# csiro-icvg/Diff3DHPE

Hardware: AMD Instinct MI355X
Metric: pose_sequences_per_sec (higher is better)
Workload: dtype f16x3

## Files before the change

diff3dhpe_amd/csrc/kernels_qkv_sattn.hip:

```cpp
#include "d3d_kernels.h"
#include "qkv_fused_kloop.h"

#include <math.h>

namespace d3d {
namespace {

#include "kloop_common.h"
#include "attn_lds.h"

QF_SHAPE(8, 3, 256, 192, 4, 3);
constexpr int QS_J = 17, QS_FPT = 15, QS_ROWS = QS_J * QS_FPT;
constexpr int QS_PLANE = QS_J * 128, QS_SLOT = 6 * QS_PLANE;
constexpr int QS_QKV = QF_STAGE;
constexpr int QS_STX = QS_QKV + 8 * QS_SLOT;
constexpr int QS_RAW = 2 * QF_STAGE;
constexpr int QS_RAW_MAX = 16384;
constexpr int QS_LDS = QS_STX + QF_BM * 8;
static_assert(QS_LDS <= 160 * 1024 && QS_RAW + QS_RAW_MAX <= QS_STX, "LDS map");
constexpr int QS_PV = 0, QS_PK = 2 * QS_PLANE, QS_PQ = 4 * QS_PLANE;

#ifndef QS_ABL
#define QS_ABL 0
#endif

struct QsArgs {
  const _Float16* Ap;
  const _Float16* Wp;
  const float* bias;
  const float* csum;
  const float* st_in;
  int st_np;
  float eps, out_scale;
  _Float16* out;
  int M, K, F, mtiles, D;
  unsigned* range;
  _Float16 *ph, *pl;
};

__device__ __forceinline__ void qs_attention(unsigned char* slot, int lane, _Float16* out_row0, int D) {
  constexpr int T = QS_J;
  unsigned char* const sVh = slot + QS_PV;
  unsigned char* const sVl = slot + QS_PV + QS_PLANE;
  unsigned char* const sKh = slot + QS_PK;
  unsigned char* const sKl = slot + QS_PK + QS_PLANE;
  unsigned char* const sQh = slot + QS_PQ;
  unsigned char* const sQl = slot + QS_PQ + QS_PLANE;
  unsigned char* const patch = slot + QS_PQ;
  const int r = lane & 31, h = lane >> 5;
  h8 qh[4], ql[4];
#pragma unroll
  for (int ks = 0; ks < 4; ++ks) {
    const int qo = kswz(r, 2 * ks + h);
    qh[ks] = *reinterpret_cast<const h8*>(sQh + qo);
    ql[ks] = *reinterpret_cast<const h8*>(sQl + qo);
  }
  f32x16 sacc;
#pragma unroll
  for (int q = 0; q < 16; ++q) sacc[q] = 0.f;
#pragma unroll
  for (int ks = 0; ks < 4; ++ks) {
    const int ko = kswz(r, 2 * ks + h);
    const h8 kh = *reinterpret_cast<const h8*>(sKh + ko);
    const h8 kl = *reinterpret_cast<const h8*>(sKl + ko);
    sacc = __builtin_amdgcn_mfma_f32_32x32x16_f16(kl, qh[ks], sacc, 0, 0, 0);
    sacc = __builtin_amdgcn_mfma_f32_32x32x16_f16(kh, ql[ks], sacc, 0, 0, 0);
    sacc = __builtin_amdgcn_mfma_f32_32x32x16_f16(kh, qh[ks], sacc, 0, 0, 0);
  }
  float m = -INFINITY;
  if (h != 0) sacc[8] = -INFINITY;
#pragma unroll
  for (int q = 0; q < 9; ++q) m = fmaxf(m, sacc[q]);
  m = fmaxf(m, __shfl_xor(m, 32, 64));
  constexpr float C_EXP = 1.4426950408889634f / 64.0f;
  const float mb = m * C_EXP;
  float l = 0.f;
#pragma unroll
  for (int q = 0; q < 16; ++q) {
    float e = 0.0f;
    if (q < 9) {
      e = __builtin_amdgcn_exp2f(fmaf(sacc[q], C_EXP, -mb));
      l += e;
    }
    sacc[q] = e;
  }
  l += __shfl_xor(l, 32, 64);
  f32x16 oacc[2];
#pragma unroll
  for (int q = 0; q < 16; ++q) { oacc[0][q] = 0.f; oacc[1][q] = 0.f; }
#pragma unroll
  for (int s2 = 0; s2 < 2; ++s2) {
    h8 eh, el;
    {
      if (s2 == 0) {
        float e8[8];
#pragma unroll
        for (int jj = 0; jj < 8; ++jj) e8[jj] = sacc[jj];
        split8_e(e8, eh, el);
      } else {
        unsigned a, b;
        split_pair_s(sacc[8], 0.0f, 1024.0f, a, b);
        u32x4 hv = {a, 0u, 0u, 0u}, lv = {b, 0u, 0u, 0u};
        eh = __builtin_bit_cast(h8, hv);
        el = __builtin_bit_cast(h8, lv);
      }
    }
    const int k0 = 16 * s2 + 4 * h;
    const int gi = lane & 15, tq_ = gi >> 2, tp_ = gi & 3;
#pragma unroll
    for (int dt = 0; dt < 2; ++dt) {
      const int d0 = dt * 32 + 16 * ((lane >> 4) & 1);
      const int ch = (d0 >> 3) + (tp_ >> 1), sub = (tp_ & 1) * 8;
      const int o0 = vswz(k0 + tq_, ch) + sub, o1 = vswz(k0 + 8 + tq_, ch) + sub;
      const s4v a0 = __builtin_amdgcn_ds_read_tr16_b64_v4i16((__attribute__((address_space(3))) s4v*)(uintptr_t)(sVh + o0));
      const s4v a1 = __builtin_amdgcn_ds_read_tr16_b64_v4i16((__attribute__((address_space(3))) s4v*)(uintptr_t)(sVh + o1));
      const s4v c0 = __builtin_amdgcn_ds_read_tr16_b64_v4i16((__attribute__((address_space(3))) s4v*)(uintptr_t)(sVl + o0));
      const s4v c1 = __builtin_amdgcn_ds_read_tr16_b64_v4i16((__attribute__((address_space(3))) s4v*)(uintptr_t)(sVl + o1));
      h8 vh, vl;
      {
        const h4 a0h = __builtin_bit_cast(h4, a0), a1h = __builtin_bit_cast(h4, a1);
        const h4 c0h = __builtin_bit_cast(h4, c0), c1h = __builtin_bit_cast(h4, c1);
#pragma unroll
        for (int e = 0; e < 4; ++e) { vh[e] = a0h[e]; vh[4 + e] = a1h[e]; vl[e] = c0h[e]; vl[4 + e] = c1h[e]; }
      }
      oacc[dt] = __builtin_amdgcn_mfma_f32_32x32x16_f16(vl, eh, oacc[dt], 0, 0, 0);
      oacc[dt] = __builtin_amdgcn_mfma_f32_32x32x16_f16(vh, el, oacc[dt], 0, 0, 0);
      oacc[dt] = __builtin_amdgcn_mfma_f32_32x32x16_f16(vh, eh, oacc[dt], 0, 0, 0);
    }
    __builtin_amdgcn_sched_barrier(0);
  }
  const float inv = 1.0f / (8192.0f * l);
  const int tqc = r < T ? r : 0;
  u32x4 pw[6];
#pragma unroll
  for (int dt = 0; dt < 2; ++dt) {
#pragma unroll
    for (int g4 = 0; g4 < 4; ++g4) {
      const int vo = vswz(tqc, dt * 4 + g4) + 8 * h;
      const uint2 vqh = *reinterpret_cast<const uint2*>(sVh + vo);
      const uint2 vql = *reinterpret_cast<const uint2*>(sVl + vo);
      float o4[4];
#pragma unroll
      for (int pr = 0; pr < 2; ++pr) {
        const unsigned ph_ = pr ? vqh.y : vqh.x, pl_ = pr ? vql.y : vql.x;
        float n0, n1;
        asm("v_fma_mix_f32 %0, %1, %2, 0 op_sel_hi:[1,0,0]" : "=v"(n0) : "v"(pl_), "v"(-0.125f));
        asm("v_fma_mix_f32 %0, %1, %2, %3 op_sel_hi:[1,0,0]" : "=v"(n0) : "v"(ph_), "v"(-0.125f), "v"(n0));
        asm("v_fma_mix_f32 %0, %1, %2, 0 op_sel:[1,0,0] op_sel_hi:[1,0,0]" : "=v"(n1) : "v"(pl_), "v"(-0.125f));
        asm("v_fma_mix_f32 %0, %1, %2, %3 op_sel:[1,0,0] op_sel_hi:[1,0,0]" : "=v"(n1) : "v"(ph_), "v"(-0.125f), "v"(n1));
        o4[2 * pr] = __builtin_fmaf(oacc[dt][4 * g4 + 2 * pr], inv, n0);
        o4[2 * pr + 1] = __builtin_fmaf(oacc[dt][4 * g4 + 2 * pr + 1], inv, n1);
      }
      unsigned h0, l0, h1, l1;
      split_pair(o4[0], o4[1], 8.0f, h0, l0);
      split_pair(o4[2], o4[3], 8.0f, h1, l1);
      const h4 oh = __builtin_bit_cast(h4, make_uint2(h0, h1)), ol = __builtin_bit_cast(h4, make_uint2(l0, l1));
      if (!(QS_ABL & 4)) patch_wr(patch, r, h, g4, oh, ol);
      else asm volatile("" ::"v"(oh), "v"(ol));
    }
    asm volatile("" ::: "memory");
#pragma unroll
    for (int it = 0; it < 3; ++it) pw[dt * 3 + it] = (QS_ABL & 4) ? u32x4{0u, 0u, 0u, 0u} : patch_rd(patch, 8 * it + (lane >> 3), lane & 7);
    asm volatile("" ::: "memory");
  }
  _Float16* const pw_ptr = out_row0 + (size_t)(lane >> 3) * 2 * D + 8 * (lane & 7);
  const size_t pw_stride = (size_t)8 * 2 * D;
#pragma unroll
  for (int it = 0; it < 3; ++it)
    if (8 * it + (lane >> 3) < T) {
#pragma unroll
      for (int dt = 0; dt < 2; ++dt) *reinterpret_cast<u32x4*>(pw_ptr + it * pw_stride + dt * 64) = pw[dt * 3 + it];
    }
}

typedef float qs_f2 __attribute__((ext_vector_type(2)));

__device__ __forceinline__ void qs_row_stats(unsigned char* lds, const QsArgs& a, int m0, int wave, int lane, bool st_dma) {
  float2* const srow = reinterpret_cast<float2*>(lds + QS_STX);
  const int K = a.K;
  if (lane < 32) {
    const int t = wave * 32 + lane, row = m0 + t;
    float sm = 0.f, sq = 0.f;
    if (row < a.M) {
      const float2* raw = st_dma ? reinterpret_cast<const float2*>(lds + QS_RAW) + t * a.st_np
                                 : reinterpret_cast<const float2*>(a.st_in) + (size_t)row * a.st_np;
      for (int p = 0; p < a.st_np; ++p) { sm += raw[p].x; sq += raw[p].y; }
    }
    if (sq >= (X3_HALF_MAX * 0.125f) * (X3_HALF_MAX * 0.125f)) range_raise(a.range, RANGE_BIT_ACT);
    const float mean = sm / (float)K;
    const float var = fmaxf(sq / (float)K - mean * mean, 0.0f);
    if (row < a.M && mean * mean > 256.0f * var) range_raise(a.range, RANGE_BIT_STATS);
    const float rstd = 1.0f / sqrtf(var + a.eps);
    srow[t] = make_float2(rstd * a.out_scale, -mean * rstd);
  }
}

__device__ __forceinline__ void qs_fold_split(const f32x4& ac, qs_f2 sx, qs_f2 sy, const float4& cs, const float4& bb, float osc, float& amax,
                                              u32x2_alias& hv, u32x2_alias& lv) {
  typedef qs_f2 f2;
  f2 a01, a23, c01, c23, b01, b23;
  a01.x = ac[0]; a01.y = ac[1]; a23.x = ac[2]; a23.y = ac[3];
  c01.x = cs.x; c01.y = cs.y; c23.x = cs.z; c23.y = cs.w;
  b01.x = bb.x; b01.y = bb.y; b23.x = bb.z; b23.y = bb.w;
  const f2 v01 = __builtin_elementwise_fma(sx, a01, __builtin_elementwise_fma(sy, c01, b01));
  const f2 v23 = __builtin_elementwise_fma(sx, a23, __builtin_elementwise_fma(sy, c23, b23));
  amax = fmaxf(fmaxf(amax, fabsf(v01.x)), fabsf(v01.y));
  amax = fmaxf(fmaxf(amax, fabsf(v23.x)), fabsf(v23.y));
  unsigned h0, l0, h1, l1;
  split_pair(v01.x, v01.y, osc, h0, l0);
  split_pair(v23.x, v23.y, osc, h1, l1);
  hv[0] = h0; hv[1] = h1; lv[0] = l0; lv[1] = l1;
}

template <bool PLANES>
__device__ __forceinline__ void qs_tail(f32x4 (&acc)[QF_TM][QF_NJ], unsigned char* lds, const QsArgs& a, int mt, int hd, int m0, int n0,
                                        int wave, int lane, int wm, int wn, int r16, int q) {
  float2 st[QF_TM];
#pragma unroll
  for (int i = 0; i < QF_TM; ++i) st[i] = reinterpret_cast<const float2*>(lds + QS_STX)[wm * 16 * QF_TM + 16 * i + r16];
  float4 cs4[QF_NJ], b4[QF_NJ];
#pragma unroll
  for (int j = 0; j < QF_NJ; ++j) {
    const int n = n0 + wn * 48 + 16 * j + 4 * q;
    cs4[j] = *reinterpret_cast<const float4*>(a.csum + n);
    b4[j] = *reinterpret_cast<const float4*>(a.bias + n);
  }
  float amaxj[QF_NJ] = {0.0f, 0.0f, 0.0f};
  typedef qs_f2 f2;
  const int chunk = 2 * wn + (q >> 1), half8 = (q & 1) << 3;
  auto write_pass = [&](int pass) {
#pragma unroll
    for (int i = 0; i < QF_TM; ++i) {
      if (pass == 0 ? (i > 4) : (i < 4 && !(wm == 1 && i == 0))) continue;
      const int R = wm * 16 * QF_TM + 16 * i + r16;
      const int fr = (R * 241) >> 12, jr = R - fr * QS_J;
      if (((fr >> 2) & 1) != pass || fr >= QS_FPT) continue;
      unsigned char* const row = lds + QS_QKV + ((fr & 3) + 4 * (fr >> 3)) * QS_SLOT + jr * 128 + half8;
      unsigned char* const pkq = row + ((chunk ^ ((jr >> 1) & 7)) << 4);
      unsigned char* const pv = row + ((chunk ^ vkey(jr)) << 4);
      const f2 sx = (f2)(st[i].x), sy = (f2)(st[i].y);
#pragma unroll
      for (int j = 0; j < QF_NJ; ++j) {
        const float osc = j == 0 ? 1.0f : 8.0f;
        u32x2_alias hv, lv;
        qs_fold_split(acc[i][j], sx, sy, cs4[j], b4[j], osc, amaxj[j], hv, lv);
        unsigned char* const ph = j == 0 ? pkq + QS_PQ : (j == 1 ? pkq + QS_PK : pv + QS_PV);
        if (!(QS_ABL & 1)) {
          *reinterpret_cast<u32x2_alias*>(ph) = hv;
          *reinterpret_cast<u32x2_alias*>(ph + QS_PLANE) = lv;
        }
      }
    }
  };
  auto attend = [&](int pass) {
    const int fr = (wave & 3) + 4 * pass + 8 * (wave >> 2);
    const long long gf = (long long)mt * QS_FPT + fr;
    if (!(QS_ABL & 2) && fr < QS_FPT && gf < a.F)
      qs_attention(lds + QS_QKV + wave * QS_SLOT, lane, a.out + ((size_t)gf * QS_J) * 2 * a.D + hd * 128, a.D);
  };
  auto range_check = [&]() {
    float amax = 0.0f;
#pragma unroll
    for (int j = 0; j < QF_NJ; ++j) amax = fmaxf(amax, amaxj[j] * (j == 0 ? 1.0f : (j == 1 ? 8.0f : 16.015f)));
    if (amax > X3_HALF_MAX) range_raise(a.range, RANGE_BIT_ACT);
  };
  if (PLANES) {
#pragma unroll
    for (int i = 0; i < QF_TM; ++i) {
      const int R = wm * 16 * QF_TM + 16 * i + r16, m = m0 + R;
      if (R >= QS_ROWS || m >= a.M) continue;
      const f2 sx = (f2)(st[i].x), sy = (f2)(st[i].y);
      const size_t o = (size_t)m * 3 * a.D + hd * 64 + 16 * wn + 4 * q;
#pragma unroll
      for (int j = 0; j < QF_NJ; ++j) {
        const float osc = j == 0 ? 1.0f : 8.0f;
        u32x2_alias hv, lv;
        qs_fold_split(acc[i][j], sx, sy, cs4[j], b4[j], osc, amaxj[j], hv, lv);
        *reinterpret_cast<u32x2_alias*>(a.ph + o + j * a.D) = hv;
        *reinterpret_cast<u32x2_alias*>(a.pl + o + j * a.D) = lv;
      }
    }
    range_check();
    return;
  }
  write_pass(0);
  __syncthreads();
  attend(0);
  __syncthreads();
  write_pass(1);
  range_check();
  __syncthreads();
  attend(1);
}

__global__ __launch_bounds__(512) void k_qkv_sattn(QsArgs a) {
  extern __shared__ __attribute__((aligned(16))) unsigned char lds[];
  const int G = (int)gridDim.x, b = (int)blockIdx.x;
  const int tiles = a.mtiles * 8;
  if (b >= tiles) return;
  const int nitems = (tiles - b + G - 1) / G;
  const int vfull = (a.mtiles / 8) * 64, mrem = a.mtiles % 8;
  auto tile_of = [&](int o, int& mt, int& hd) {
    if (o < vfull) {
      const int xcd = o & 7, slot = o >> 3;
      mt = (slot >> 3) * 8 + xcd;
      hd = slot & 7;
    } else {
      const int o2 = o - vfull;
      mt = (a.mtiles / 8) * 8 + o2 % mrem;
      hd = o2 / mrem;
    }
  };

  const int K = a.K;
  const size_t K2 = 2 * (size_t)K;
  const int nk = K / 32;
  int mt = 0, hd = 0;
  tile_of(b, mt, hd);
  QF_STAGE_FIRST(a.Ap, a.Wp, mt * QS_ROWS, hd * QF_BN)
  int tid_o = (int)threadIdx.x;
  for (int item = 0; item < nitems; ++item) {
    QF_TILE_LANES;
    QF_TILE_NEXT(mtn, hdn);
    const int m0 = mt * QS_ROWS, n0 = hd * QF_BN;

    const int st_bytes = QF_BM * a.st_np * 8;
    const bool st_dma = st_bytes <= QS_RAW_MAX && (((size_t)m0 * a.st_np * 8) & 15) == 0;
    int st_issued = 0;
    if (st_dma) {
      const char* src = reinterpret_cast<const char*>(a.st_in + (size_t)m0 * a.st_np * 2);
#pragma unroll
      for (int it = 0; it < QS_RAW_MAX / 1024 / 8; ++it) {
        const int pc = wave + it * 8;
        if (pc * 1024 < st_bytes) {
          KL_GLDS(sgpr_ptr(src + pc * 1024) + lane * 16, QS_RAW + pc * 1024);
          ++st_issued;
        }
      }
    }

    QF_TILE_PLAN(a.Ap, a.Wp, m0, n0, mtn * QS_ROWS, hdn * QF_BN);
    QF_TILE_ACC;
    int issued_prev = st_issued;
    QF_KLOOP_HEAD(QF_PIECE)
    qs_row_stats(lds, a, m0, wave, lane, st_dma);
    QF_KLOOP_TAIL(QF_PIECE)
    __builtin_amdgcn_s_setprio(0);

    __syncthreads();

    qs_tail<false>(acc, lds, a, mt, hd, m0, n0, wave, lane, wm, wn, r16, q);
    mt = mtn; hd = hdn;
    __syncthreads();
  }
}

struct QdSrc {
  const float *x2d, *y;
  const float *G, *P, *Q;
  int q_stride;
  int TJ, y_bcast_T;
};
constexpr int QD_GROW = 8;
constexpr int QD_QSLOTS = 16;
constexpr int QD_G = 0, QD_P = QD_G + QF_BN * QD_GROW * 4, QD_Q = QD_P + QS_J * QF_BN * 4;
static_assert(QD_Q + QD_QSLOTS * QF_BN * 4 <= QS_QKV, "the direct form's tables fit the unused stage area");
static_assert(QF_BM <= QD_QSLOTS * QS_J, "a tile's rows span at most QD_QSLOTS frames, so at most QD_QSLOTS batch elements");

__device__ __forceinline__ int qd_col(int c, int hd) { return 512 * ((c % 48) >> 4) + 64 * hd + 16 * (c / 48) + (c & 15); }

template <int CIN2>
__device__ __forceinline__ void qd_stage(unsigned char* lds, const QdSrc& d, int M, int m0, int hd, int tid) {
  constexpr int CIN = CIN2 + 3;
  float* const sG = reinterpret_cast<float*>(lds + QD_G);
  float* const sP = reinterpret_cast<float*>(lds + QD_P);
  float* const sQ = reinterpret_cast<float*>(lds + QD_Q);
  for (int idx = tid; idx < QF_BN * CIN; idx += 512) {
    const int c = idx / CIN, k = idx - c * CIN;
    sG[c * QD_GROW + k] = d.G[QF_BN * CIN * hd + idx];
  }
  for (int idx = tid; idx < QS_J * QF_BN; idx += 512) {
    const int j = idx / QF_BN, c = idx - j * QF_BN;
    sP[idx] = d.P[j * 1536 + QF_BN * hd + c];
  }
  if (d.Q) {
    const int b_lo = m0 / d.TJ, nb = d.q_stride ? min(QD_QSLOTS, M / d.TJ - b_lo) : 1;
    for (int idx = tid; idx < nb * QF_BN; idx += 512) {
      const int sl = idx / QF_BN, c = idx - sl * QF_BN;
      sQ[idx] = d.Q[(size_t)(b_lo + sl) * d.q_stride + qd_col(c, hd)];
    }
  }
}

template <int CIN2>
__device__ __forceinline__ void qd_fill(f32x4 (&acc)[QF_TM][QF_NJ], const unsigned char* lds, const QdSrc& d, int M, int m0, int wm, int wn,
                                        int r16, int q) {
  constexpr int CIN = CIN2 + 3;
  const int c0 = wn * 48 + 4 * q;
  const int b_lo = m0 / d.TJ;
  const float* const sG = reinterpret_cast<const float*>(lds + QD_G);
  const float* const sP = reinterpret_cast<const float*>(lds + QD_P);
  const float* const sQ = reinterpret_cast<const float*>(lds + QD_Q);
  float u[QF_TM][CIN];
#pragma unroll
  for (int ii = 0; ii < QF_TM; ++ii) {
    const int R = wm * 16 * QF_TM + 16 * ii + r16, m = m0 + R;
    const int fr = (R * 241) >> 12, jr = R - fr * QS_J;
#pragma unroll
    for (int k = 0; k < CIN; ++k) u[ii][k] = 0.0f;
    if (m < M) {
#pragma unroll
      for (int k = 0; k < CIN2; ++k) u[ii][k] = d.x2d[(size_t)m * CIN2 + k];
      const size_t my = d.y_bcast_T ? ((size_t)(m / d.TJ) * QS_J + jr) : (size_t)m;
#pragma unroll
      for (int k = 0; k < 3; ++k) u[ii][CIN2 + k] = d.y[my * 3 + k];
    }
  }
#pragma unroll
  for (int j = 0; j < QF_NJ; ++j) {
#pragma unroll
    for (int e = 0; e < 4; ++e) {
      float g[CIN];
#pragma unroll
      for (int k = 0; k < CIN; ++k) g[k] = sG[(c0 + 16 * j + e) * QD_GROW + k];
#pragma unroll
      for (int ii = 0; ii < QF_TM; ++ii) {
        float v = 0.0f;
#pragma unroll
        for (int k = 0; k < CIN; ++k) v = fmaf(u[ii][k], g[k], v);
        acc[ii][j][e] = v;
      }
      __builtin_amdgcn_sched_barrier(0);
    }
  }
#pragma unroll
  for (int i = 0; i < QF_TM; ++i) {
    const int R = wm * 16 * QF_TM + 16 * i + r16, m = m0 + R;
    const int po = (R - ((R * 241) >> 12) * QS_J) * QF_BN + c0;
    const int qo = c0 + (d.q_stride ? min(m / d.TJ - b_lo, QD_QSLOTS - 1) * QF_BN : 0);
    if (m < M) {
#pragma unroll
      for (int j = 0; j < QF_NJ; ++j) {
        const float4 p4 = *reinterpret_cast<const float4*>(sP + po + 16 * j);
        acc[i][j][0] += p4.x; acc[i][j][1] += p4.y; acc[i][j][2] += p4.z; acc[i][j][3] += p4.w;
      }
      if (d.Q) {
#pragma unroll
        for (int j = 0; j < QF_NJ; ++j) {
          const float4 q4 = *reinterpret_cast<const float4*>(sQ + qo + 16 * j);
          acc[i][j][0] += q4.x; acc[i][j][1] += q4.y; acc[i][j][2] += q4.z; acc[i][j][3] += q4.w;
        }
      }
    }
    __builtin_amdgcn_sched_barrier(0);
  }
}

template <int CIN2, bool PLANES>
__global__ __launch_bounds__(512) void k_qkv_sattn_direct(QsArgs a, QdSrc d) {
  extern __shared__ __attribute__((aligned(16))) unsigned char lds[];
  const int G = (int)gridDim.x, b = (int)blockIdx.x;
  const int tiles = a.mtiles * 8;
  if (b >= tiles) return;
  const int nitems = (tiles - b + G - 1) / G;
  KL_XCD_TILE_ORDER(a.mtiles, 8);
  int tid_o = (int)threadIdx.x;
  for (int item = 0; item < nitems; ++item) {
    QF_TILE_LANES;
    int mt = 0, hd = 0;
    tile_of(item * G + b, mt, hd);
    const int m0 = mt * QS_ROWS, n0 = hd * QF_BN;
    qd_stage<CIN2>(lds, d, a.M, m0, hd, tid);
    qs_row_stats(lds, a, m0, wave, lane, false);
    __syncthreads();
    f32x4 acc[QF_TM][QF_NJ];
    qd_fill<CIN2>(acc, lds, d, a.M, m0, wm, wn, r16, q);
    __builtin_amdgcn_sched_barrier(0);
    qs_tail<PLANES>(acc, lds, a, mt, hd, m0, n0, wave, lane, wm, wn, r16, q);
    __syncthreads();
  }
}

}

bool qkv_sattn_ok(int J, int D, int H, int K) { return J == QS_J && H == 8 && D == 512 && K % 64 == 0 && K >= 128; }

hipError_t launch_qkv_sattn(const void* Apair, const void* Wpair_headmajor, const float* bias_hm, const float* csum_hm, const float* st_in,
                            int st_np, float eps, int w_exp, void* out_x3, int M, int K, int J, int D, int H, hipStream_t s) {
  if (!qkv_sattn_ok(J, D, H, K) || M <= 0 || M % J != 0 || st_np < 1 || !Apair || !Wpair_headmajor || !bias_hm || !csum_hm || !st_in || !out_x3)
    return hipErrorInvalidValue;
  if (w_exp < -14 || w_exp > 12) return hipErrorInvalidValue;
  QsArgs a{};
  a.Ap = (const _Float16*)Apair; a.Wp = (const _Float16*)Wpair_headmajor; a.bias = bias_hm; a.csum = csum_hm; a.st_in = st_in;
  a.st_np = st_np; a.eps = eps; a.out_scale = ldexpf(1.0f, -(3 + w_exp));
  a.out = (_Float16*)out_x3; a.M = M; a.K = K; a.F = M / J; a.mtiles = (a.F + QS_FPT - 1) / QS_FPT; a.D = D;
  a.range = launch_range_word();
  int grid = 0;
  if (hipError_t ge = persistent_grid((long long)a.mtiles * 8, grid)) return ge;
  return launch_lds<k_qkv_sattn>(dim3(grid), dim3(512), QS_LDS, s, a);
}

bool qkv_sattn_direct_ok(int J, int D, int H, int in_chans) { return qkv_sattn_ok(J, D, H, D) && in_chans >= 1 && in_chans <= 3; }

hipError_t launch_qkv_sattn_direct(const float* x2d, const float* y, int y_bcast_T, int in_chans, const float* G, const float* P, const float* Q,
                                   int q_stride, const float* bias_hm, const float* csum_hm, const float* st_in, int st_np, float eps, void* out_x3,
                                   void* planes_hi, void* planes_lo, int M, int T, int J, int D, int H, hipStream_t s) {
  if (!qkv_sattn_direct_ok(J, D, H, in_chans) || M <= 0 || T <= 0 || M % (T * J) != 0 || st_np < 1 || !x2d || !y || !G || !P || !bias_hm || !csum_hm ||
      !st_in || (q_stride != 0 && q_stride != 3 * D) || (!out_x3 && (!planes_hi || !planes_lo)))
    return hipErrorInvalidValue;
  QsArgs a{};
  a.bias = bias_hm; a.csum = csum_hm; a.st_in = st_in; a.st_np = st_np; a.eps = eps; a.out_scale = 1.0f;
  a.out = (_Float16*)out_x3; a.M = M; a.K = D; a.F = M / J; a.mtiles = (a.F + QS_FPT - 1) / QS_FPT; a.D = D;
  a.ph = (_Float16*)planes_hi; a.pl = (_Float16*)planes_lo;
  a.range = launch_range_word();
  QdSrc d{};
  d.x2d = x2d; d.y = y; d.G = G; d.P = P; d.Q = Q; d.q_stride = q_stride; d.TJ = T * J; d.y_bcast_T = y_bcast_T;
  int grid = 0;
  if (hipError_t ge = persistent_grid((long long)a.mtiles * 8, grid)) return ge;
#define D3D_QD(C2)                                                                                                      \
  case C2:                                                                                                              \
    return out_x3 ? launch_lds<k_qkv_sattn_direct<C2, false>>(dim3(grid), dim3(512), QS_LDS, s, a, d)                   \
                  : launch_lds<k_qkv_sattn_direct<C2, true>>(dim3(grid), dim3(512), QS_LDS, s, a, d);
  switch (in_chans) {
    D3D_QD(1) D3D_QD(2) D3D_QD(3)
  }
#undef D3D_QD
  return hipErrorInvalidValue;
}

}
```

Baseline: 136.1.

## Prefetch direct-form inputs into double-buffered LDS via async global-to-LDS loads

The direct QKV kernel now issues global_load_lds requests for the next tile's x2d, y and row-statistic partials into one of two LDS input buffers while the current tile computes. qd_fill and qs_row_stats then read those inputs from LDS instead of global memory. Per-head G/P tables are restaged only when the head changes, and the broadcast Q row is split from the per-batch Q rows. The goal is to hide global load latency and cut redundant table reloads, at the cost of more LDS use, clamped index logic and a wait_vm(0) that drains every outstanding load each iteration.

```diff
diff --git a/diff3dhpe_amd/csrc/kernels_qkv_sattn.hip b/diff3dhpe_amd/csrc/kernels_qkv_sattn.hip
--- a/diff3dhpe_amd/csrc/kernels_qkv_sattn.hip
+++ b/diff3dhpe_amd/csrc/kernels_qkv_sattn.hip
@@ -175,14 +175,14 @@
 
 typedef float qs_f2 __attribute__((ext_vector_type(2)));
 
-__device__ __forceinline__ void qs_row_stats(unsigned char* lds, const QsArgs& a, int m0, int wave, int lane, bool st_dma) {
+__device__ __forceinline__ void qs_row_stats(unsigned char* lds, const QsArgs& a, int m0, int wave, int lane, bool st_dma, int raw_off = QS_RAW) {
   float2* const srow = reinterpret_cast<float2*>(lds + QS_STX);
   const int K = a.K;
   if (lane < 32) {
     const int t = wave * 32 + lane, row = m0 + t;
     float sm = 0.f, sq = 0.f;
     if (row < a.M) {
-      const float2* raw = st_dma ? reinterpret_cast<const float2*>(lds + QS_RAW) + t * a.st_np
+      const float2* raw = st_dma ? reinterpret_cast<const float2*>(lds + raw_off) + t * a.st_np
                                  : reinterpret_cast<const float2*>(a.st_in) + (size_t)row * a.st_np;
       for (int p = 0; p < a.st_np; ++p) { sm += raw[p].x; sq += raw[p].y; }
     }
@@ -364,13 +364,22 @@
 constexpr int QD_GROW = 8;
 constexpr int QD_QSLOTS = 16;
 constexpr int QD_G = 0, QD_P = QD_G + QF_BN * QD_GROW * 4, QD_Q = QD_P + QS_J * QF_BN * 4;
-static_assert(QD_Q + QD_QSLOTS * QF_BN * 4 <= QS_QKV, "the direct form's tables fit the unused stage area");
+constexpr int QD_STNP_MAX = 2;
+constexpr int QD_IN = QD_Q + QD_QSLOTS * QF_BN * 4;
+constexpr int QD_IN_X = 0, QD_IN_Y = QD_IN_X + QF_BM * 3 * 4, QD_IN_ST = QD_IN_Y + QF_BM * 3 * 4;
+constexpr int QD_IN_BYTES = QD_IN_ST + QF_BM * QD_STNP_MAX * 8;
+static_assert(QD_IN + 2 * QD_IN_BYTES <= QS_QKV, "the direct form's tables and input buffers fit the unused stage area");
+static_assert(QS_QKV + 8 * QS_SLOT <= QS_STX && QS_STX + QF_BM * 8 <= QS_LDS, "frame slots and row statistics lie behind them");
+static_assert(QD_IN % 16 == 0 && QD_IN_BYTES % 16 == 0 && QD_IN_Y % 16 == 0 && QD_IN_ST % 16 == 0, "input blocks start on 16 bytes");
 static_assert(QF_BM <= QD_QSLOTS * QS_J, "a tile's rows span at most QD_QSLOTS frames, so at most QD_QSLOTS batch elements");
 
+#define QD_GLDS4(SRC, DSTOFF)                                                                                            \
+  __builtin_amdgcn_global_load_lds(reinterpret_cast<const char*>(SRC), (__attribute__((address_space(3))) void*)(uintptr_t)(lds + (DSTOFF)), 4, 0, 0)
+
 __device__ __forceinline__ int qd_col(int c, int hd) { return 512 * ((c % 48) >> 4) + 64 * hd + 16 * (c / 48) + (c & 15); }
 
 template <int CIN2>
-__device__ __forceinline__ void qd_stage(unsigned char* lds, const QdSrc& d, int M, int m0, int hd, int tid) {
+__device__ __forceinline__ void qd_stage_tables(unsigned char* lds, const QdSrc& d, int hd, int tid) {
   constexpr int CIN = CIN2 + 3;
   float* const sG = reinterpret_cast<float*>(lds + QD_G);
   float* const sP = reinterpret_cast<float*>(lds + QD_P);
@@ -383,37 +392,70 @@
     const int j = idx / QF_BN, c = idx - j * QF_BN;
     sP[idx] = d.P[j * 1536 + QF_BN * hd + c];
   }
-  if (d.Q) {
-    const int b_lo = m0 / d.TJ, nb = d.q_stride ? min(QD_QSLOTS, M / d.TJ - b_lo) : 1;
-    for (int idx = tid; idx < nb * QF_BN; idx += 512) {
-      const int sl = idx / QF_BN, c = idx - sl * QF_BN;
-      sQ[idx] = d.Q[(size_t)(b_lo + sl) * d.q_stride + qd_col(c, hd)];
-    }
+  if (d.Q && !d.q_stride && tid < QF_BN) sQ[tid] = d.Q[qd_col(tid, hd)];
+}
+
+__device__ __forceinline__ void qd_stage_q_rows(unsigned char* lds, const QdSrc& d, int M, int m0, int hd, int tid) {
+  float* const sQ = reinterpret_cast<float*>(lds + QD_Q);
+  const int b_lo = m0 / d.TJ, nb = min(QD_QSLOTS, M / d.TJ - b_lo);
+  for (int idx = tid; idx < nb * QF_BN; idx += 512) {
+    const int sl = idx / QF_BN, c = idx - sl * QF_BN;
+    sQ[idx] = d.Q[(size_t)(b_lo + sl) * d.q_stride + qd_col(c, hd)];
   }
 }
 
 template <int CIN2>
-__device__ __forceinline__ void qd_fill(f32x4 (&acc)[QF_TM][QF_NJ], const unsigned char* lds, const QdSrc& d, int M, int m0, int wm, int wn,
-                                        int r16, int q) {
+__device__ __forceinline__ void qd_request(unsigned char* lds, const QsArgs& a, const QdSrc& d, int m0, int buf, bool st_lds, int wave, int lane) {
+  constexpr int NPX = QF_BM * CIN2 / 64, NPY = QF_BM * 3 / 64;
+  const int base = QD_IN + buf * QD_IN_BYTES, M = a.M;
+#pragma unroll
+  for (int it = 0; it < (NPX + NPY + 7) / 8; ++it) {
+    const int p = wave + 8 * it;
+    if (p < NPX) {
+      const int e = min(m0 * CIN2 + p * 64 + lane, M * CIN2 - 1);
+      QD_GLDS4(d.x2d + e, base + QD_IN_X + p * 256);
+    } else if (p < NPX + NPY) {
+      const int ey = (p - NPX) * 64 + lane;
+      int e;
+      if (d.y_bcast_T) {
+        const int R = ey / 3, k = ey - 3 * R, m = min(m0 + R, M - 1);
+        e = ((m / d.TJ) * QS_J + (R - ((R * 241) >> 12) * QS_J)) * 3 + k;
+      } else {
+        e = min(m0 * 3 + ey, M * 3 - 1);
+      }
+      QD_GLDS4(d.y + e, base + QD_IN_Y + (p - NPX) * 256);
+    }
+  }
+  if (st_lds) {
+    for (int p = 0; p < a.st_np; ++p) {
+      const int e = min((m0 + wave * 32) * a.st_np * 2 + p * 64 + lane, M * a.st_np * 2 - 1);
+      QD_GLDS4(a.st_in + e, base + QD_IN_ST + (wave * a.st_np + p) * 256);
+    }
+  }
+}
+
+template <int CIN2>
+__device__ __forceinline__ void qd_fill(f32x4 (&acc)[QF_TM][QF_NJ], const unsigned char* lds, const QdSrc& d, int M, int m0, int in_off, int wm,
+                                        int wn, int r16, int q) {
   constexpr int CIN = CIN2 + 3;
   const int c0 = wn * 48 + 4 * q;
   const int b_lo = m0 / d.TJ;
   const float* const sG = reinterpret_cast<const float*>(lds + QD_G);
   const float* const sP = reinterpret_cast<const float*>(lds + QD_P);
   const float* const sQ = reinterpret_cast<const float*>(lds + QD_Q);
+  const float* const sX = reinterpret_cast<const float*>(lds + in_off + QD_IN_X);
+  const float* const sY = reinterpret_cast<const float*>(lds + in_off + QD_IN_Y);
   float u[QF_TM][CIN];
 #pragma unroll
   for (int ii = 0; ii < QF_TM; ++ii) {
     const int R = wm * 16 * QF_TM + 16 * ii + r16, m = m0 + R;
-    const int fr = (R * 241) >> 12, jr = R - fr * QS_J;
 #pragma unroll
     for (int k = 0; k < CIN; ++k) u[ii][k] = 0.0f;
     if (m < M) {
 #pragma unroll
-      for (int k = 0; k < CIN2; ++k) u[ii][k] = d.x2d[(size_t)m * CIN2 + k];
-      const size_t my = d.y_bcast_T ? ((size_t)(m / d.TJ) * QS_J + jr) : (size_t)m;
-#pragma unroll
-      for (int k = 0; k < 3; ++k) u[ii][CIN2 + k] = d.y[my * 3 + k];
+      for (int k = 0; k < CIN2; ++k) u[ii][k] = sX[R * CIN2 + k];
+#pragma unroll
+      for (int k = 0; k < 3; ++k) u[ii][CIN2 + k] = sY[R * 3 + k];
     }
   }
 #pragma unroll
@@ -465,16 +507,30 @@
   const int nitems = (tiles - b + G - 1) / G;
   KL_XCD_TILE_ORDER(a.mtiles, 8);
   int tid_o = (int)threadIdx.x;
+  int hd_tab = -1;
+  const bool st_lds = a.st_np <= QD_STNP_MAX;
   for (int item = 0; item < nitems; ++item) {
     QF_TILE_LANES;
     int mt = 0, hd = 0;
     tile_of(item * G + b, mt, hd);
     const int m0 = mt * QS_ROWS, n0 = hd * QF_BN;
-    qd_stage<CIN2>(lds, d, a.M, m0, hd, tid);
-    qs_row_stats(lds, a, m0, wave, lane, false);
+    const int in_off = QD_IN + (item & 1) * QD_IN_BYTES;
+    if (item == 0) qd_request<CIN2>(lds, a, d, m0, 0, st_lds, wave, lane);
+    if (hd != hd_tab) {
+      qd_stage_tables<CIN2>(lds, d, hd, tid);
+      hd_tab = hd;
+    }
+    if (d.Q && d.q_stride) qd_stage_q_rows(lds, d, a.M, m0, hd, tid);
+    wait_vm(0);
+    qs_row_stats(lds, a, m0, wave, lane, st_lds, in_off + QD_IN_ST);
     __syncthreads();
+    if (item + 1 < nitems) {
+      int mtn = 0, hdn = 0;
+      tile_of((item + 1) * G + b, mtn, hdn);
+      qd_request<CIN2>(lds, a, d, mtn * QS_ROWS, (item + 1) & 1, st_lds, wave, lane);
+    }
     f32x4 acc[QF_TM][QF_NJ];
-    qd_fill<CIN2>(acc, lds, d, a.M, m0, wm, wn, r16, q);
+    qd_fill<CIN2>(acc, lds, d, a.M, m0, in_off, wm, wn, r16, q);
     __builtin_amdgcn_sched_barrier(0);
     qs_tail<PLANES>(acc, lds, a, mt, hd, m0, n0, wave, lane, wm, wn, r16, q);
     __syncthreads();
```

After: 136.5 (median of 6 runs). No clear change (+0.3%).
